# Chairy-neko/TinyRayTracing

Hardware: AMD Instinct MI355X
Metric: Mrays/s (higher is better)
Workload: dtype f32; 1 GPU; example-scenes-cg22 test/back Cornell-style box (26 triangles), 1920x1080, 256 spp; scene=back, width=1920, height=1080, spp=256, triangles=26, bvh_nodes=4, bvh_builder=auto, leaf_num=8, inner_node_bytes=64, overlap_passes=False, fixed_nee=False, tiling=single GPU

## Files before the change

tinyraytracing_amd/csrc/trt_api.hip:

```cpp
#include <hip/hip_runtime.h>

#include <dlfcn.h>

#include <algorithm>
#include <cstdio>
#include <cstdlib>
#include <atomic>
#include <limits>
#include <chrono>
#include <cstring>
#include <condition_variable>
#include <memory>
#include <mutex>
#include <string>
#include <thread>
#include <vector>

#include "trt.h"
#include "trt_kernels.h"
#include "trt_wide.h"
#include "trt_oct_build.h"
#include "trt_denoise_kernels.h"
#include "trt_reproject_kernels.h"
#include "trt_refit_kernels.h"
// ... 18 lines not shown
    } while (0)

constexpr uint32_t MAX_TRACE_BLOCKS = 8192;
constexpr uint32_t SPILL_STRIDE = MAX_TRACE_BLOCKS * TRT_TRACE_BLOCK;
constexpr uint32_t MAX_BOUNCES = TRT_MAX_PATH_DEPTH + 2;
constexpr uint32_t COUNT_STRIDE = (MAX_BOUNCES + 2 + 1023u) & ~1023u;
constexpr uint32_t COUNT_ROW_MIN = 16;
inline uint32_t countRows(uint32_t nl) { return std::max(COUNT_ROW_MIN, (nl + 3u + 15u) & ~15u); }
inline unsigned long long* pairCounter(uint32_t* d_counts, uint32_t rows, uint32_t b) { return reinterpret_cast<unsigned long long*>(d_counts + (size_t)(rows - 2u) * COUNT_STRIDE) + b; }
static_assert(TRT_MAX_SCENE_LIGHTS <= 65535u, "counter area");
constexpr uint32_t MAX_BVH_DEPTH = 256;
#ifndef TRT_DEFAULT_NODE_KIND
#define TRT_DEFAULT_NODE_KIND 1
#endif

struct DevBuf {
    void* p = nullptr;
    size_t bytes = 0;
    int ensure(size_t need)
    {
        if (need <= bytes) return TRT_OK;
        if (p) { (void)hipFree(p); p = nullptr; bytes = 0; }
        HIPC(hipMalloc(&p, need));
        bytes = need;
        return TRT_OK;
    }
    void release()
    {
        if (p) (void)hipFree(p);
        p = nullptr;
        bytes = 0;
    }
};

}

struct trt_handle {
    int device = 0;
    SceneDev sc{};
    std::vector<void*> scene_allocs;
    std::vector<uint32_t> light_mats;
    std::vector<LightBox> light_boxes;
    uint32_t depth = 0;
    uint32_t bvh2_depth = 0;
    uint32_t shade_tabs = 0;
    uint32_t shade_pad_lds = 0;
    const void* lds_image = nullptr;
    uint32_t lds_image_bytes = 0;
    uint32_t lds_tab[5] = {0, 0, 0, 0, 0};
    int trace_impl = 3;
    bool slim_walk = false;
    bool hit8 = false;
    bool bin_walk = false;
    int node_kind = 0;
    uint32_t oct_levels = 0;
    bool dbg = false;
    uint32_t rays_per_wave = 256, fill_blocks = 2048, max_blocks = 8192;
    uint32_t traceGrid(uint32_t n) const
    {
        uint32_t b = (n + TRT_TRACE_BLOCK - 1) / TRT_TRACE_BLOCK;
        if (rays_per_wave > 64) {
            const uint32_t want = (uint32_t)(((uint64_t)n + 4ull * rays_per_wave - 1) / (4ull * rays_per_wave));
            b = std::min(b, std::max(fill_blocks, want));
        }
        b = std::min(std::max(b, 8u), std::min(max_blocks, 8192u));
        return (b + 7u) & ~7u;
    }
    uint32_t tail_n = 131072;
    DevBuf arena, spill, small_buf, out_buf, io_buf;
    size_t spill_words_per_slot = 0;
    hipStream_t slot_streams[2] = {nullptr, nullptr};
    int n_slots = 2;
    uint32_t* pinned_counts = nullptr;
    uint32_t count_rows = COUNT_ROW_MIN;
    uint32_t slot_seq[2] = {0, 0};
    int fail_at_bounce = -1;
    std::vector<hipEvent_t> events;
    uint32_t n_materials = 0, n_light_tris = 0, n_tri_trav = 0;
    bool light_boxes_fixed = false;
    struct Refit {
        bool ready = false;
        DevBuf order2, order4, order8, exact8, small;
        std::vector<uint32_t> level2, level4, level8;
        DevBuf light_of_mat;
        hipEvent_t ev[4] = {};
    } refit;
    ~trt_handle()
    {
        refit.order2.release();
        refit.order4.release();
        refit.order8.release();
        refit.exact8.release();
        refit.small.release();
        refit.light_of_mat.release();
        for (hipEvent_t e : refit.ev)
            if (e) (void)hipEventDestroy(e);
        for (void* p : scene_allocs) (void)hipFree(p);
        arena.release();
        spill.release();
        small_buf.release();
        out_buf.release();
        io_buf.release();
        for (hipEvent_t e : events) (void)hipEventDestroy(e);
        for (hipStream_t st : slot_streams) if (st) (void)hipStreamDestroy(st);
        if (pinned_counts) (void)hipHostFree(pinned_counts);
    }
// ... 169 lines not shown
using ShadeKernel = void (*)(SceneDev, ShadeArgs);
using TailKernel = void (*)(SceneDev, TailArgs);

enum Walk { WALK_UNIFORM, WALK_UNIFORM_FLAGS, WALK_UNIFORM_HIT8, WALK_OCT, WALK_WIDE16, WALK_WIDE_SPILL, N_WALKS };
struct Traversal {
    Walk closest, occlusion;
    bool binned;
};
Traversal traversalOf(const trt_handle* h)
{
    if (h->trace_impl == 0) return {h->hit8 ? WALK_UNIFORM_HIT8 : WALK_UNIFORM, h->slim_walk ? WALK_UNIFORM_FLAGS : WALK_UNIFORM, h->bin_walk};
    const Walk w = h->node_kind == 1 ? WALK_OCT : (h->depth <= 16 ? WALK_WIDE16 : WALK_WIDE_SPILL);
    return {w, w, h->bin_walk};
}
struct ClosestRow { ClosestKernel k[2][3], query; bool redo; };
struct ShadowRow { ShadowKernel k[2]; ClosestKernel query; bool redo; };
template <class D>
ClosestRow closestRow()
{
    return {{{k_trace_closest<false, D, 0>, k_trace_closest<false, D, 1>, k_trace_closest<false, D, PRIMARY_LIST>},
             {k_trace_closest<true, D, 0>, k_trace_closest<true, D, 1>, k_trace_closest<true, D, PRIMARY_LIST>}},
            k_trace_query<D, QUERY_CLOSEST>, D::REDO};
}
template <class D>
ShadowRow shadowRow()
{
    return {{k_trace_shadow<false, D>, k_trace_shadow<true, D>}, k_trace_query<D, QUERY_OCCLUDED>, D::REDO};
}
const ClosestRow closest_rows[N_WALKS] = {closestRow<WalkUniform>(), {}, closestRow<WalkUniformHit8>(), closestRow<WalkOct>(), closestRow<WalkWide16>(), closestRow<WalkWideSpill>()};
const ShadowRow shadow_rows[N_WALKS] = {shadowRow<WalkUniform>(), shadowRow<WalkUniformFlags>(), {}, shadowRow<WalkOct>(), shadowRow<WalkWide16>(), shadowRow<WalkWideSpill>()};
ClosestKernel closestKernel(const trt_handle* h, bool count, int primary)
{
    const Traversal t = traversalOf(h);
    if (t.binned && primary == 0) return count ? k_trace_closest_binned<true> : k_trace_closest_binned<false>;
    return closest_rows[t.closest].k[count][primary];
}
ShadowKernel shadowKernel(const trt_handle* h, bool count) { return shadow_rows[traversalOf(h).occlusion].k[count]; }
FixKernel fixKernel(const trt_handle* h, bool shadow, int primary)
{
    const FixKernel k[4] = {k_trace_fix<false, 0>, k_trace_fix<false, 1>, k_trace_fix<false, PRIMARY_LIST>, k_trace_fix<true, 0>};
    const Traversal t = traversalOf(h);
    return (shadow ? shadow_rows[t.occlusion].redo : closest_rows[t.closest].redo) ? k[shadow ? 3 : primary] : nullptr;
}
ClosestKernel queryKernel(const trt_handle* h, int query)
{
    const Traversal t = traversalOf(h);
    return query == QUERY_OCCLUDED ? shadow_rows[t.occlusion].query : closest_rows[t.closest].query;
}
FixKernel queryFixKernel(const trt_handle* h, int query)
{
    if (!fixKernel(h, query == QUERY_OCCLUDED, 0)) return nullptr;
    return query == QUERY_OCCLUDED ? k_trace_fix<true, 0, QUERY_OCCLUDED> : k_trace_fix<false, 0, QUERY_CLOSEST>;
}
ShadeKernel shadeKernel(uint32_t tabs, int lights, bool list, bool hit8)
{
    if (hit8) {
        const ShadeKernel s[2][3] = {
            {k_shade<31u, SHADE_ONE, false, TRT_SHADE1_BLOCK, TRT_SHADE1_WAVES, true>, k_shade<31u, SHADE_FEW, false, TRT_SHADEN_BLOCK, TRT_SHADEN_WAVES, true>,
             k_shade<31u, SHADE_MANY, false, TRT_SHADEN_BLOCK, TRT_SHADEN_WAVES, true>},
            {k_shade<31u, SHADE_ONE, true, TRT_SHADE1_BLOCK, TRT_SHADE1_WAVES, true>, k_shade<31u, SHADE_FEW, true, TRT_SHADEN_BLOCK, TRT_SHADEN_WAVES, true>,
             k_shade<31u, SHADE_MANY, true, TRT_SHADEN_BLOCK, TRT_SHADEN_WAVES, true>}};
        return s[list][lights];
    }
    const ShadeKernel k[5][2][3] = {
        {{k_shade<31u, SHADE_ONE>, k_shade<31u, SHADE_FEW>, k_shade<31u, SHADE_MANY>}, {k_shade<31u, SHADE_ONE, true>, k_shade<31u, SHADE_FEW, true>, k_shade<31u, SHADE_MANY, true>}},
        {{k_shade<15u, SHADE_ONE>, k_shade<15u, SHADE_FEW>, k_shade<15u, SHADE_MANY>}, {k_shade<15u, SHADE_ONE, true>, k_shade<15u, SHADE_FEW, true>, k_shade<15u, SHADE_MANY, true>}},
        {{k_shade<7u, SHADE_ONE>, k_shade<7u, SHADE_FEW>, k_shade<7u, SHADE_MANY>}, {k_shade<7u, SHADE_ONE, true>, k_shade<7u, SHADE_FEW, true>, k_shade<7u, SHADE_MANY, true>}},
        {{k_shade<3u, SHADE_ONE>, k_shade<3u, SHADE_FEW>, k_shade<3u, SHADE_MANY>}, {k_shade<3u, SHADE_ONE, true>, k_shade<3u, SHADE_FEW, true>, k_shade<3u, SHADE_MANY, true>}},
        {{k_shade<0u, SHADE_ONE>, k_shade<0u, SHADE_FEW>, k_shade<0u, SHADE_MANY>}, {k_shade<0u, SHADE_ONE, true>, k_shade<0u, SHADE_FEW, true>, k_shade<0u, SHADE_MANY, true>}}};
    return k[tabs == 31u ? 0 : (tabs == 15u ? 1 : (tabs == 7u ? 2 : (tabs == 3u ? 3 : 4)))][list][lights];
}
TailKernel tailKernel(bool count, bool list)
{
    if (list) return count ? k_tail<true, true> : k_tail<false, true>;
    return count ? k_tail<true> : k_tail<false>;
}

void launchTraceClosest(const trt_handle* h, ClosestKernel k, FixKernel fix, hipStream_t stream, uint32_t* spill, const RaySource& src, f4* hit, uint32_t n,
                        DeviceStats* d_stats, RedoList redo)
{
    const dim3 b(TRT_TRACE_BLOCK);
    hipLaunchKernelGGL(k, dim3(h->traceGrid(n)), b, 0, stream, h->sc, src, hit, n, spill, SPILL_STRIDE, d_stats, redo);
    if (fix) hipLaunchKernelGGL(fix, dim3(TRT_FIX_BLOCKS), b, 0, stream, h->sc, src, hit, (const f4*)nullptr, 0u, (f4*)nullptr, spill, SPILL_STRIDE, redo, 0u, d_stats);
}

void launchTraceShadow(const trt_handle* h, ShadowKernel k, FixKernel fix, hipStream_t stream, uint32_t* spill, const ShadowQueue& sq, uint32_t n, uint32_t light_mat,
                       f4* Lacc, DeviceStats* d_stats, uint32_t any, RedoList redo, const LightBox& lbox)
{
    const dim3 b(TRT_TRACE_BLOCK);
    hipLaunchKernelGGL(k, dim3(h->traceGrid(n)), b, 0, stream, h->sc, sq, n, light_mat, Lacc, spill, SPILL_STRIDE, d_stats, any, redo, lbox);
    if (!fix) return;
    const RaySource src{sq.sa, sq.sb, TileDesc{}, 0u};
    hipLaunchKernelGGL(fix, dim3(TRT_FIX_BLOCKS), b, 0, stream, h->sc, src, (f4*)nullptr, (const f4*)sq.sw, light_mat, Lacc, spill, SPILL_STRIDE, redo, any, d_stats);
}

}

namespace {
struct SceneImage {
    const trt_scene* s = nullptr;
    unsigned threads = 1;
    bool dbg = false;
    uint32_t bvh2_depth = 0;
    int trace_impl = 3;
    int node_kind = 0;
    std::vector<TriIsect> isect;
// ... 206 lines not shown
    if (im.cum_monotone)
        if (int e = upload(h.get(), im.cum.data(), im.cum.size(), &h->sc.light_cum)) return e;
    if (int e = upload(h.get(), im.tex.data(), im.tex.size(), &h->sc.textures)) return e;
    if (int e = upload(h.get(), im.tex_bytes.data(), im.tex_bytes.size(), &h->sc.tex_bytes)) return e;
    lap("uploads");
    h->sc.n_tris = s->n_tris;
    h->sc.n_nodes = s->n_nodes;
    h->sc.n_lights = s->n_lights;
    h->n_materials = s->n_materials;
    h->n_light_tris = s->n_light_tris;
    if (const char* e = std::getenv("TRT_SHADOW_STOP")) h->light_boxes_fixed = std::atoi(e) == 0;
    h->sc.light0_area = s->n_lights ? s->lights[0].area : 0.0f;
    h->sc.leaf_alpha = im.leaf_alpha;
    h->sc.cull_alpha = im.cull_alpha;
    h->sc.cam = s->camera;
    for (uint32_t i = 0; i < s->n_lights; ++i) h->light_mats.push_back((uint32_t)s->lights[i].mat);
    {
        const uint32_t want[5] = {(uint32_t)(s->n_materials * sizeof(MaterialDev)), (uint32_t)(s->n_lights * sizeof(LightDev)),
                                  h->sc.light_cum ? (uint32_t)(s->n_light_tris * sizeof(float)) : 0u, (uint32_t)(s->n_light_tris * sizeof(LightTriDev)),
                                  s->n_tris <= 64 ? (uint32_t)(s->n_tris * sizeof(TriShade)) : 0u};
        uint32_t used = 0;
        for (int k = 0; k < 5; ++k) {
            const uint32_t padded = (want[k] + 15u) & ~15u;
            if (want[k] && used + padded <= TRT_SHADE_LDS_TABLE_BYTES) { h->lds_tab[k] = want[k]; used += padded; }
        }
        if (std::getenv("TRT_SHADE_NO_LDS")) h->lds_tab[0] = h->lds_tab[1] = h->lds_tab[2] = h->lds_tab[3] = h->lds_tab[4] = 0;
        if (std::getenv("TRT_SHADE_NO_LDS_TRIS")) h->lds_tab[4] = 0;
        uint32_t have = 0;
        for (int k = 0; k < 5; ++k) have |= h->lds_tab[k] ? (1u << k) : 0u;
        h->shade_tabs = 0;
        for (uint32_t m : {31u, 15u, 7u, 3u})
            if ((have & m) == m) { h->shade_tabs = m; break; }
        if (im.dbg)
            std::fprintf(stderr, "trt_create: k_shade tables %u (lds bytes: materials %u, lights %u, cdf %u, light tris %u, shading tris %u)\n", h->shade_tabs,
                         h->lds_tab[0], h->lds_tab[1], h->lds_tab[2], h->lds_tab[3], h->lds_tab[4]);
        size_t total = 0;
        for (int k = 0; k < 5; ++k)
            if (h->shade_tabs >> k & 1u) total += (h->lds_tab[k] + 15u) & ~15u;
        if (total) {
            void* img = nullptr;
            HIPC(hipMalloc(&img, total));
            h->scene_allocs.push_back(img);
            h->lds_image = img;
            h->lds_image_bytes = (uint32_t)total;
            if (int e = packLdsImage(h.get(), nullptr)) return e;
        }
    }
    h->slim_walk = h->trace_impl == 0 && s->n_tris <= 64;
    if (const char* e = std::getenv("TRT_SLIM_WALK")) h->slim_walk = h->slim_walk && std::atoi(e) != 0;
    h->hit8 = h->slim_walk && h->shade_tabs == 31u;
    h->bin_walk = h->hit8;
    if (const char* e = std::getenv("TRT_BIN_WALK")) h->bin_walk = h->bin_walk && std::atoi(e) != 0;
    if (im.dbg) std::fprintf(stderr, "trt_create: slim walk %d, 8-byte hit records %d, binned walk %d\n", (int)h->slim_walk, (int)h->hit8, (int)h->bin_walk);

    const uint32_t stack_levels = std::max(h->depth, h->bvh2_depth + 2u);
    uint32_t spill_levels = stack_levels > (uint32_t)TRT_LDS_STACK_MAX ? stack_levels - TRT_LDS_STACK_MAX + 1 : 1;
    if (h->node_kind == 1 && h->oct_levels > OCT_LDS_LEVELS) spill_levels = std::max(spill_levels, 2u * (h->oct_levels - OCT_LDS_LEVELS + 1));
    h->spill_words_per_slot = (size_t)spill_levels * SPILL_STRIDE;
    if (int e = h->spill.ensure(h->spill_words_per_slot * 2 * sizeof(uint32_t))) return e;
    for (hipStream_t& st : h->slot_streams) HIPC(hipStreamCreateWithFlags(&st, hipStreamNonBlocking));
    h->count_rows = countRows(h->sc.n_lights);
    const size_t pinned_words = 2 * (2 * (size_t)h->count_rows + 16);
    HIPC(hipHostMalloc((void**)&h->pinned_counts, pinned_words * sizeof(uint32_t), hipHostMallocDefault));
    std::memset(h->pinned_counts, 0, pinned_words * sizeof(uint32_t));
    if (const char* e = std::getenv("TRT_SLOTS")) h->n_slots = std::atoi(e) >= 2 ? 2 : 1;
    if (const char* e = std::getenv("TRT_TEST_FAIL_AT_BOUNCE")) h->fail_at_bounce = std::atoi(e);
    if (const char* e = std::getenv("TRT_SHADE_PAD_LDS")) {
        h->shade_pad_lds = std::min(100000u, (uint32_t)std::strtoul(e, nullptr, 10));
        for (uint32_t tabs : {31u, 15u, 7u, 3u, 0u})
            for (bool list : {false, true})
                for (int lights : {SHADE_ONE, SHADE_FEW, SHADE_MANY})
                    for (bool hit8 : {false, true})
                        if (!hit8 || tabs == 31u)
                            (void)hipFuncSetAttribute(reinterpret_cast<const void*>(shadeKernel(tabs, lights, list, hit8)), hipFuncAttributeMaxDynamicSharedMemorySize, (int)h->shade_pad_lds);
    }

    *out = h.release();
    return TRT_OK;
}
}

extern "C" {

const char* trt_last_error(void) { return g_err.c_str(); }
int trt_abi_version(void) { return TRT_ABI_VERSION; }

int trt_rows_selected(const trt_params* p)
{
    if (!p) return -1;
    int n = 0;
    for (int y = p->y0; y < p->y1; ++y) n += rowSelected(p, y) ? 1 : 0;
    return n;
}

int trt_create(const trt_scene* s, int device, trt_handle** out)
{
    if (!s || !out) return fail(TRT_EINVAL, "trt_create: null argument");
    *out = nullptr;
    SceneImage im;
    if (int e = buildSceneImage(s, im)) return e;
    return createOnDevice(im, device, out);
}

void trt_destroy(trt_handle* h)
{
    if (!h) return;
    (void)hipSetDevice(h->device);
    delete h;
}

namespace {
constexpr int N_SLOTS = 2;
struct PassSlot {
    hipStream_t stream = nullptr;
    RayQueue Q[2];
    f4* hit = nullptr;
    f4* Lacc = nullptr;
    ShadowArena shadow{nullptr, 0};
    uint32_t* d_counts = nullptr;
    uint32_t* host_counts = nullptr;
    uint32_t seq = 0;
    uint32_t* spill = nullptr;
    RedoList redo{nullptr, nullptr};
    enum State { IDLE, PACK, PACKWAIT, ISSUE, WAIT, RESOLVE } state = IDLE;
    uint32_t chunk = 0, s0 = 0, sc_count = 0, n_active = 0, b = 0;
    int cur = 0;
};
// ... 203 lines not shown
        if (d_sq) HIPC(hipMemcpyAsync(d_sq, in.sumsq, acc_bytes, hipMemcpyHostToDevice, stream));
    }
    if (!in.list || in.rays) return TRT_OK;
    uint32_t list_max = 0;
    hipLaunchKernelGGL(k_list_max, dim3(std::min<uint32_t>((in.npix + 255) / 256, 1024u)), dim3(256), 0, stream, in.host ? (const uint32_t*)d_table : in.pixels, in.npix, d_list_max);
    HIPC(hipMemcpyAsync(&list_max, d_list_max, sizeof(list_max), hipMemcpyDeviceToHost, stream));
    HIPC(hipStreamSynchronize(stream));
    if ((uint64_t)list_max >= (uint64_t)p->width * (uint64_t)p->height) return fail(TRT_EINVAL, "pixel list holds an entry >= width * height");
    return TRT_OK;
}

int renderCore(trt_handle* h, const trt_params* p, uint32_t s_begin, uint32_t s_end, const RenderInput& in, hipStream_t stream, trt_stats* stats_out)
{
    const uint32_t n_samples = s_end - s_begin, npix = in.npix, nl = h->sc.n_lights, count_rows = h->count_rows;
    PassPlan plan;
    if (int e = planArena(h, p, npix, n_samples, in.list, renderFootprint(nl), plan)) return e;
    const size_t counts_bytes = (size_t)COUNT_STRIDE * count_rows * sizeof(uint32_t), acc_bytes = (size_t)npix * 3 * sizeof(double);
    const bool own_table = in.host || (in.rays && !in.pixels);
    const size_t table_bytes = !own_table ? 0 : (in.list ? (size_t)npix * sizeof(uint32_t) : in.rows.size() * sizeof(int32_t));
    Layout L;
    const size_t o_table = L.add(table_bytes, 256), o_counts = L.add(counts_bytes * N_SLOTS, 256);
    const size_t o_stats = L.add(sizeof(DeviceStats), 256), o_redo = L.add(2 * N_SLOTS * sizeof(uint32_t), 64), o_list_max = L.add(sizeof(uint32_t), 64);
    const size_t o_pack = L.add(N_SLOTS * sizeof(unsigned long long), 64);
    const size_t o_sum = L.add(in.host ? acc_bytes : 0, 256), o_sumsq = L.add(in.host && in.sumsq ? acc_bytes : 0, sizeof(double));
    if (int e = h->small_buf.ensure(L.bytes)) return e;
    char* sb = (char*)h->small_buf.p;
    DeviceStats* d_stats = (DeviceStats*)(sb + o_stats);
    const void* d_table = own_table ? (const void*)(sb + o_table) : (const void*)in.pixels;
    double* d_sum = in.host ? (double*)(sb + o_sum) : in.sum;
    double* d_sq = !in.sumsq ? nullptr : (in.host ? (double*)(sb + o_sumsq) : in.sumsq);
    HIPC(hipMemsetAsync(d_stats, 0, o_sum - o_stats, stream));
    if (int e = stageInput(in, p, sb + o_table, table_bytes, d_sum, d_sq, (uint32_t*)(sb + o_list_max), stream)) return e;
    PassSlot slots[N_SLOTS];
    for (int k = 0; k < plan.slots; ++k) {
        PassSlot& S = slots[k];
        S.stream = h->slot_streams[k];
        SlotLayout::carve(S, (f4*)((char*)h->arena.p + plan.slot_bytes * (size_t)k), plan.N, nl);
        S.redo.count = (uint32_t*)(sb + o_redo) + 2 * k;
        S.d_counts = (uint32_t*)(sb + o_counts + counts_bytes * (size_t)k);
        S.host_counts = h->pinned_counts + (size_t)k * (2 * count_rows + 16);
        S.seq = h->slot_seq[k];
        S.spill = (uint32_t*)h->spill.p + (size_t)k * h->spill_words_per_slot;
    }
    const int lights = nl == 1u ? SHADE_ONE : (nl <= (uint32_t)TRT_MAX_LIGHTS ? SHADE_FEW : SHADE_MANY);
    const uint32_t shade_block = lights == SHADE_ONE ? (uint32_t)TRT_SHADE1_BLOCK : (uint32_t)TRT_SHADEN_BLOCK;
    const uint32_t rows_lds = (in.rows.size() <= shadeRowsLds((int)shade_block) && p->height <= 65536) ? (uint32_t)in.rows.size() : 0u;
    const bool count = (p->flags & TRT_FLAG_COUNT) != 0;
    const int camera = in.list ? PRIMARY_LIST : 1;
    const ClosestKernel camera_k = closestKernel(h, count, camera), queue_k = closestKernel(h, count, 0);
    const FixKernel camera_fix = fixKernel(h, false, camera), queue_fix = fixKernel(h, false, 0), shadow_fix = fixKernel(h, true, 0);
    const ShadowKernel shadow_k = shadowKernel(h, count);
    const ShadeKernel shade_k = shadeKernel(h->shade_tabs, lights, in.list, h->hit8);
    const TailKernel tail_k = tailKernel(count, in.list);
    const ShadeArgs shade_args = shadeArgsOf(h, p, in, d_table, rows_lds, d_stats);
    const TileDesc& td = shade_args.td;
    if (h->dbg)
        std::fprintf(stderr, "%s: k_shade %s, rows in lds %u, grid_ok %u\n", in.rays ? "trt_render_rays" : (in.list ? "trt_render_pixels" : "trt_render"),
                     lights == SHADE_ONE ? "one" : (lights == SHADE_FEW ? "few" : "many"), rows_lds, td.grid_ok);

    Timer tm{h, (p->flags & TRT_FLAG_TIMING) != 0};
    trt_stats st;
    std::memset(&st, 0, sizeof(st));
    hipEvent_t ev_begin = tm.get(0), ev_end = tm.get(1), ev_resolved = tm.get(2);
    if (!ev_begin || !ev_end || !ev_resolved) return fail(TRT_EHIP, "hipEventCreate failed");
    HIPC(hipEventRecord(ev_begin, stream));
    Drain drain{h, slots, plan.slots, stream};
    for (int k = 0; k < plan.slots; ++k) HIPC(hipStreamWaitEvent(slots[k].stream, ev_begin, 0));

    uint32_t next_chunk = 0, resolved_upto = 0;
    auto startPass = [&](PassSlot& S) -> int {
        if (next_chunk >= plan.n_chunks) { S.state = PassSlot::IDLE; return TRT_OK; }
        S.chunk = next_chunk++;
        S.s0 = s_begin + S.chunk * plan.chunk;
        S.sc_count = std::min(plan.chunk, s_end - S.s0);
        S.n_active = npix * S.sc_count;
        S.b = 0;
        S.cur = 0;
        HIPC(hipMemsetAsync(S.d_counts, 0, counts_bytes, S.stream));
        if (!in.rays) st.rays_camera += S.n_active;
        S.state = in.rays ? PassSlot::PACK : PassSlot::ISSUE;
        return TRT_OK;
    };
    auto issuePack = [&](PassSlot& S) -> int {
        const size_t at = (size_t)(S.s0 - s_begin) * npix * 3, comps = (size_t)S.n_active * 3;
        const float* org = in.org + at;
        const float* dir = in.dir + at;
        if (in.host) {
            float* stage = (float*)S.Q[1].ra;
            HIPC(hipMemcpyAsync(stage, org, comps * sizeof(float), hipMemcpyHostToDevice, S.stream));
            HIPC(hipMemcpyAsync(stage + comps, dir, comps * sizeof(float), hipMemcpyHostToDevice, S.stream));
            org = stage;
            dir = stage + comps;
        }
        unsigned long long* packed = (unsigned long long*)(sb + o_pack) + (&S - slots);
        HIPC(hipMemsetAsync(packed, 0, sizeof(*packed), S.stream));
        tm.launch(TRT_K_GEN_PRIMARY, S.stream, st, [&] {
            hipLaunchKernelGGL(k_rays_pack, dim3(std::min<uint32_t>((S.n_active + 255) / 256, 65536u)), dim3(256), 0, S.stream, org, dir, S.n_active, S.Q[0], S.Lacc,
                               (uint32_t*)packed);
        });
        S.seq++;
        hipLaunchKernelGGL(k_publish_counts, dim3(1), dim3(64), 0, S.stream, S.d_counts, COUNT_STRIDE, 0u, 1u, packed, (volatile uint32_t*)S.host_counts, 2u * count_rows, S.seq);
        S.state = PassSlot::PACKWAIT;
        return TRT_OK;
    };
    auto completePack = [&](PassSlot& S) -> int {
        if (int e = awaitCounts(S, count_rows)) return e;
        const uint32_t n_valid = S.host_counts[1];
        if (n_valid > S.n_active) return fail(TRT_EHIP, "internal error: more rays queued than given");
        st.rays_camera += n_valid;
        S.n_active = n_valid;
        S.state = n_valid ? PassSlot::ISSUE : PassSlot::RESOLVE;
        return TRT_OK;
    };
    auto issueFront = [&](PassSlot& S) -> int {
        const RaySource src{S.Q[S.cur].ra, S.Q[S.cur].rb, td, S.s0};
        tm.launch(TRT_K_TRACE_CLOSEST, S.stream, st, [&] {
            const bool generated = S.b == 0 && !in.rays;
            launchTraceClosest(h, generated ? camera_k : queue_k, generated ? camera_fix : queue_fix, S.stream, S.spill, src, S.hit, S.n_active, d_stats, S.redo);
        });
        ShadeArgs A = shade_args;
        A.qin = S.Q[S.cur];
        A.hit = S.hit;
        A.n = S.n_active;
        A.qout = S.Q[S.cur ^ 1];
        if (lights == SHADE_MANY) A.sq_arena = S.shadow;
        else
            for (uint32_t l = 0; l < (uint32_t)TRT_MAX_LIGHTS; ++l) A.sq[l] = l < nl ? S.shadow.queue(l) : ShadowQueue{nullptr, nullptr, nullptr};
        A.pair_count = pairCounter(S.d_counts, count_rows, S.b);
        A.shadow_counts = S.d_counts + (size_t)COUNT_STRIDE + S.b;
        A.Lacc = S.Lacc;
        A.s0 = S.s0;
        A.primary = (S.b == 0 && !in.rays) ? 1u : 0u;
        tm.launch(TRT_K_SHADE, S.stream, st, [&] {
            hipLaunchKernelGGL(shade_k, dim3(std::min<uint32_t>((S.n_active + shade_block - 1) / shade_block, 65536u)), dim3(shade_block), h->shade_pad_lds, S.stream, h->sc, A);
        });
        S.seq++;
        const uint32_t publish_block = std::min(1024u, (2u * (1u + nl) + 63u) & ~63u);
        hipLaunchKernelGGL(k_publish_counts, dim3(1), dim3(publish_block), 0, S.stream, S.d_counts, COUNT_STRIDE, S.b, 1u + nl,
                           pairCounter(S.d_counts, count_rows, S.b), (volatile uint32_t*)S.host_counts, 2u * count_rows, S.seq);
        S.state = PassSlot::WAIT;
        if (h->fail_at_bounce >= 0 && (int)S.b == h->fail_at_bounce) {
            h->fail_at_bounce = -1;
            return fail(TRT_EHIP, "injected failure (TRT_TEST_FAIL_AT_BOUNCE)");
        }
        return TRT_OK;
    };
    auto completeBounce = [&](PassSlot& S) -> int {
        if (int e = awaitCounts(S, count_rows)) return e;
        for (uint32_t l = 0; l < nl; ++l) {
            const uint32_t ns = S.host_counts[2 * (1 + l)];
            if (ns > S.n_active) return fail(TRT_EHIP, "internal error: shadow queue longer than its input");
            if (!ns) continue;
            tm.launch(TRT_K_TRACE_SHADOW, S.stream, st, [&] {
                launchTraceShadow(h, shadow_k, shadow_fix, S.stream, S.spill, S.shadow.queue(l), ns, h->light_mats[l], S.Lacc, d_stats, td.fixed_nee, S.redo, h->light_boxes[l]);
            });
            st.rays_shadow += ns;
        }
        const uint32_t n_next = S.host_counts[1];
        if (n_next > S.n_active) return fail(TRT_EHIP, "internal error: queue grew");
        st.rays_indirect += n_next;
        S.n_active = n_next;
        S.cur ^= 1;
        S.b++;
        if (S.n_active > 0 && (S.n_active <= h->tail_n || S.b >= MAX_BOUNCES)) {
            const TailArgs TA{S.Q[S.cur], S.n_active, S.Lacc, td, S.s0, p->max_depth, S.spill, SPILL_STRIDE, h->trace_impl == 0 ? 1u : 0u, d_stats};
            tm.launch(TRT_K_TAIL, S.stream, st, [&] { hipLaunchKernelGGL(tail_k, dim3(tailGrid(S.n_active)), dim3(TRT_TRACE_BLOCK), 0, S.stream, h->sc, TA); });
            S.n_active = 0;
        }
        S.state = S.n_active ? PassSlot::ISSUE : PassSlot::RESOLVE;
        return TRT_OK;
    };
    auto tryResolve = [&](PassSlot& S) -> int {
        if (S.chunk != resolved_upto) return TRT_OK;
        if (resolved_upto > 0) HIPC(hipStreamWaitEvent(S.stream, ev_resolved, 0));
        tm.launch(TRT_K_RESOLVE, S.stream, st, [&] {
            const dim3 rg(std::min<uint32_t>((npix + 255) / 256, 65536u)), rb(256);
            if (d_sq) hipLaunchKernelGGL(k_resolve_moments, rg, rb, 0, S.stream, S.Lacc, d_sum, d_sq, npix, S.sc_count, (float)p->spp);
            else hipLaunchKernelGGL(k_resolve, rg, rb, 0, S.stream, S.Lacc, d_sum, npix, S.sc_count, (float)p->spp);
        });
        HIPC(hipEventRecord(ev_resolved, S.stream));
        resolved_upto++;
        return startPass(S);
    };

    for (int k = 0; k < plan.slots; ++k)
        if (int e = startPass(slots[k])) return e;
    for (;;) {
// ... 1432 lines not shown
```

tinyraytracing_amd/csrc/trt_kernels.h:

```cpp
#pragma once
#include <hip/hip_runtime.h>
#include <type_traits>

#include "trt_path.h"
#include "trt_oct.h"

namespace trtd {

#ifndef TRT_TRACE_MINWAVES
#define TRT_TRACE_MINWAVES 0
#endif
#if TRT_TRACE_MINWAVES > 0
#define TRT_TRACE_BOUNDS __launch_bounds__(256, TRT_TRACE_MINWAVES)
#else
#define TRT_TRACE_BOUNDS __launch_bounds__(256)
#endif
constexpr int TRT_TRACE_BLOCK = 256;
#ifndef TRT_LDS_STACK_MAX_LEVELS
#define TRT_LDS_STACK_MAX_LEVELS 16
#endif
constexpr int TRT_LDS_STACK_MAX = TRT_LDS_STACK_MAX_LEVELS;
#ifndef TRT_SHADE1_BLOCK
#define TRT_SHADE1_BLOCK 512
#endif
// ... 1028 lines not shown
    uint32_t n;
    RayQueue qout;
    union {
        ShadowQueue sq[TRT_MAX_LIGHTS];
        ShadowArena sq_arena;
    };
    unsigned long long* pair_count;
    uint32_t* shadow_counts;
    uint32_t shadow_count_stride;
    f4* Lacc;
    TileDesc td;
    uint32_t s0;
    int32_t max_depth;
    uint32_t primary;
    uint32_t lds_mat_bytes, lds_light_bytes, lds_cum_bytes, lds_ltri_bytes, lds_tshade_bytes;
    const f4* lds_image;
    uint32_t lds_image_words;
    uint32_t rows_lds;
    DeviceStats* stats;
};

constexpr uint32_t TRT_SHADE_LDS_TABLE_BYTES = 24 * 1024;
constexpr uint32_t shadeRowsLds(int block) { return block >= 512 ? 8192u : 2304u; }

struct RowsShade {
    const uint16_t* lds;
    bool in_lds;
    __device__ int operator()(const TileDesc& td, uint32_t r) const
    {
        int y = 0;
        if (in_lds) {
            y = lds[r];
#if defined(__HIP_DEVICE_COMPILE__)
            asm volatile("" : "+v"(y));
#endif
        } else {
            y = td.rows[r];
        }
        return y;
    }
};

__device__ __forceinline__ void hitBarycentrics(const TriIsect* isect, const f4& ra, const f4& rb, f4& hit4)
{
    const int32_t tri = (int32_t)f2u(hit4.y);
    float u = 0.f, v = 0.f;
    if (tri >= 0) {
        float t, un, vn, det;
        if (triTest(isect[tri], mk3(ra.x, ra.y, ra.z), mk3(ra.w, rb.x, rb.y), t, un, vn, det)) { u = un / det; v = vn / det; }
    }
    hit4.z = u;
    hit4.w = v;
}
template <int LIGHTS>
__device__ inline ShadowQueue shadeQueue(const ShadeArgs& A, uint32_t li)
{
    if (LIGHTS == SHADE_MANY) return A.sq_arena.queue(li);
    return A.sq[li];
}
template <uint32_t TABS, int LIGHTS, bool LIST = false, int BLOCK = (LIGHTS == SHADE_ONE ? TRT_SHADE1_BLOCK : TRT_SHADEN_BLOCK),
          int WAVES = (LIGHTS == SHADE_ONE ? TRT_SHADE1_WAVES : TRT_SHADEN_WAVES), bool HIT8 = false>
__global__ __launch_bounds__(BLOCK, WAVES) void k_shade(SceneDev sc, ShadeArgs A)
{
    constexpr int TRT_SHADE_BLOCK = BLOCK;
    constexpr uint32_t TRT_SHADE_ROWS_LDS = shadeRowsLds(BLOCK);
    __shared__ uint32_t s_cnt[3 * (TRT_SHADE_BLOCK / 64 + 1)];
    __shared__ uint32_t s_cnt2[2 * (2 * (TRT_SHADE_BLOCK / 64) + 2)];
    __shared__ uint32_t s_shaded, s_depth;
    __shared__ __attribute__((aligned(16))) uint32_t s_tab[TABS ? TRT_SHADE_LDS_TABLE_BYTES / 4 : 4];
    __shared__ uint16_t s_rows[LIST ? 1 : TRT_SHADE_ROWS_LDS];
    __shared__ __attribute__((aligned(16))) uint32_t s_isect[HIT8 ? 64 * 12 : 4];
    const TriIsect* isect = reinterpret_cast<const TriIsect*>(s_isect);
    if (threadIdx.x == 0) { s_shaded = 0; s_depth = 0; }
    if (!LIST)
        for (uint32_t r = threadIdx.x; r < A.rows_lds; r += TRT_SHADE_BLOCK) s_rows[r] = (uint16_t)A.td.rows[r];
    std::conditional_t<LIST, PixelList, RowsShade> rows;
    if constexpr (!LIST) {
        rows.lds = s_rows;
        rows.in_lds = A.rows_lds != 0u;
    }
    bool rows_visible = A.rows_lds == 0u;
    {
        uint32_t off = 0;
        auto at = [&](uint32_t bytes) -> const void* { const void* q = s_tab + off / 4; off += (bytes + 15u) & ~15u; return q; };
        if (TABS & 1u) sc.materials = static_cast<const MaterialDev*>(at(A.lds_mat_bytes));
        if (TABS & 2u) sc.lights = static_cast<const LightDev*>(at(A.lds_light_bytes));
        if (TABS & 4u) sc.light_cum = static_cast<const float*>(at(A.lds_cum_bytes));
        if (TABS & 8u) sc.light_tris = static_cast<const LightTriDev*>(at(A.lds_ltri_bytes));
        if (TABS & 16u) sc.tri_shade = static_cast<const TriShade*>(at(A.lds_tshade_bytes));
    }
    bool staged = TABS == 0u && !HIT8;
    int parity = 0, parity2 = 0;
    uint32_t bounce_depth = 0;
    const uint32_t per_grid = gridDim.x * TRT_SHADE_BLOCK;
    auto loadTile = [&](uint32_t i, f4& hit4, f4& ra, f4& rb, f4& bt) {
        hit4 = mk4(TRT_INF, u2f(0xFFFFFFFFu), 0.0f, 0.0f); ra = mk4(0, 0, 0, 0); rb = ra; bt = mk4(1.0f, 1.0f, 1.0f, 0.0f);
        if (i < A.n) {
            if (HIT8) {
                const trt_v2f h = TRT_LDQ2(1, reinterpret_cast<const trt_v2f*>(A.hit) + i);
                hit4.x = h.x; hit4.y = h.y;
            } else {
                hit4 = TRT_LDQ(1, A.hit + i);
            }
            if (!A.primary) { ra = TRT_LDQ(1, A.qin.ra + i); rb = TRT_LDQ(1, A.qin.rb + i); bt = TRT_LDQ(1, A.qin.bt + i); }
        }
    };
#if TRT_SHADE_PIPE
    f4 n_hit, n_ra, n_rb, n_bt;
    loadTile(blockIdx.x * TRT_SHADE_BLOCK + threadIdx.x, n_hit, n_ra, n_rb, n_bt);
#endif
    for (uint32_t base = blockIdx.x * TRT_SHADE_BLOCK; base < A.n; base += per_grid) {
        const uint32_t i = base + threadIdx.x;
        f4 hit4, ra, rb, bt;
#if TRT_SHADE_PIPE
        hit4 = n_hit; ra = n_ra; rb = n_rb; bt = n_bt;
#else
        loadTile(i, hit4, ra, rb, bt);
#endif
        if (!staged || !rows_visible) {
            if (!staged) {
                f4* l = reinterpret_cast<f4*>(s_tab);
                if (TABS)
                    for (uint32_t w = threadIdx.x; w < A.lds_image_words; w += TRT_SHADE_BLOCK) l[w] = A.lds_image[w];
                if (HIT8) {
                    f4* li = reinterpret_cast<f4*>(s_isect);
                    const uint32_t words = 3u * (sc.n_tris < 64u ? sc.n_tris : 64u);
                    for (uint32_t w = threadIdx.x; w < words; w += TRT_SHADE_BLOCK) li[w] = reinterpret_cast<const f4*>(sc.tri_isect)[w];
                }
            }
            __syncthreads();
            staged = true;
            rows_visible = true;
        }
#if defined(__HIP_DEVICE_COMPILE__)
        asm volatile("" : "+v"(hit4.x), "+v"(ra.x), "+v"(rb.x), "+v"(bt.x));
#endif
#if TRT_SHADE_PIPE
        loadTile(i + per_grid, n_hit, n_ra, n_rb, n_bt);
#endif
        ShadeCtx c;
        c.had_hit = c.shade_ok = c.add_L = false;
        if (i < A.n) {
            if (A.primary) {
                primaryRay(sc, A.td, A.s0, i, ra, rb, rows);
                if (HIT8) hitBarycentrics(isect, ra, rb, hit4);
                shadeBegin(sc, A.td, A.s0, ra, rb, bt, hit4, c, rows);
                A.Lacc[i] = c.add_L ? mk4(0.0f + c.addL.x, 0.0f + c.addL.y, 0.0f + c.addL.z, 0.0f) : mk4(0.0f, 0.0f, 0.0f, 0.0f);
            } else {
                if (HIT8) hitBarycentrics(isect, ra, rb, hit4);
                shadeBegin(sc, A.td, A.s0, ra, rb, bt, hit4, c, rows);
                if (c.add_L) {
                    f4 L = A.Lacc[c.pid];
                    L.x = L.x + c.addL.x; L.y = L.y + c.addL.y; L.z = L.z + c.addL.z;
                    A.Lacc[c.pid] = L;
                }
            }
            if (c.had_hit) bounce_depth = c.depth + 1u > bounce_depth ? c.depth + 1u : bounce_depth;
        }
        const unsigned long long ok_ballot = ballotb(c.shade_ok);
        if ((threadIdx.x & 63u) == 0 && ok_ballot) atomicAdd(&s_shaded, (uint32_t)__popcll(ok_ballot));

        uint32_t pend_base = 0;
        const uint32_t* pend_s = nullptr;
        bool pend_emit = false;
        uint32_t pend_rank = 0, pend_li = 0;
        f3 pend_wo = mk3(0, 0, 0), pend_w = mk3(0, 0, 0);
        float pend_tmax = TRT_INF;
        const uint32_t nl = LIGHTS == SHADE_ONE ? 1u : sc.n_lights;
        for (uint32_t li = 0; li + 1 < nl; ++li) {
            bool emit = false;
            f3 wo = mk3(0, 0, 0), contrib = mk3(0, 0, 0);
            float t_max = TRT_INF;
            if (c.shade_ok) emit = lightSample(sc, c.vx, *c.m, li, c.rng, wo, contrib, A.td.fixed_nee != 0u, t_max);
            uint32_t rank;
            uint32_t* s = blockStage<TRT_SHADE_BLOCK>(emit, A.shadow_counts + (size_t)li * A.shadow_count_stride, s_cnt, parity, rank, pend_s, pend_base);
            parity = parity == 2 ? 0 : parity + 1;
            if (pend_emit) {
                const uint32_t slot = pend_s[TRT_SHADE_BLOCK / 64] + pend_s[threadIdx.x >> 6] + pend_rank;
                const f3 so = rayOrigin(c, pend_wo);
                TRT_STQ(2, shadeQueue<LIGHTS>(A, pend_li).sa + slot, mk4(so.x, so.y, so.z, pend_wo.x));
                TRT_STQ(2, shadeQueue<LIGHTS>(A, pend_li).sb + slot, mk4(pend_wo.y, pend_wo.z, u2f(c.pid), pend_tmax));
                TRT_STQ(2, shadeQueue<LIGHTS>(A, pend_li).sw + slot, mk4(pend_w.x, pend_w.y, pend_w.z, 0.0f));
            }
            pend_s = s; pend_emit = emit; pend_rank = rank; pend_li = li; pend_wo = wo; pend_w = c.beta * contrib; pend_tmax = t_max;
        }
        bool emit_s = false;
        f3 wo_s = mk3(0, 0, 0), w_s = mk3(0, 0, 0);
        float tmax_s = TRT_INF;
        if (nl && c.shade_ok) {
            f3 contrib = mk3(0, 0, 0);
            emit_s = lightSample(sc, c.vx, *c.m, nl - 1u, c.rng, wo_s, contrib, A.td.fixed_nee != 0u, tmax_s);
            w_s = c.beta * contrib;
        }
        NextPlan plan;
        const bool emit_next = shadeNextDecide(c, A.max_depth, plan);
        uint32_t rank_next, rank_s;
// ... 454 lines not shown
```

Measured before the change: 23940 Mrays/s.

## Fuse primary-ray closest-hit traversal into the bounce-0 shade kernel

For single-light scenes on the slim 8-byte-hit path, bounce 0 no longer launches a separate closest-hit trace kernel. The shade kernel regenerates the camera ray, walks the small BVH itself with a wave-uniform reachability mask, and shades the hit directly. This removes one kernel launch per pass along with the hit-buffer write and read round trip. In exchange it adds traversal register pressure to the shade kernel, and it reads triangles from global memory instead of the LDS copy.

```diff
diff --git a/tinyraytracing_amd/csrc/trt_api.hip b/tinyraytracing_amd/csrc/trt_api.hip
--- a/tinyraytracing_amd/csrc/trt_api.hip
+++ b/tinyraytracing_amd/csrc/trt_api.hip
@@ -94,6 +94,7 @@
     bool slim_walk = false;
     bool hit8 = false;
     bool bin_walk = false;
+    bool fuse_primary = false;
     int node_kind = 0;
     uint32_t oct_levels = 0;
     bool dbg = false;
@@ -369,6 +370,7 @@
     if (!fixKernel(h, query == QUERY_OCCLUDED, 0)) return nullptr;
     return query == QUERY_OCCLUDED ? k_trace_fix<true, 0, QUERY_OCCLUDED> : k_trace_fix<false, 0, QUERY_CLOSEST>;
 }
+ShadeKernel fusedShadeKernel() { return k_shade<31u, SHADE_ONE, false, TRT_SHADE1_BLOCK, TRT_SHADE1_WAVES, true, true>; }
 ShadeKernel shadeKernel(uint32_t tabs, int lights, bool list, bool hit8)
 {
     if (hit8) {
@@ -681,6 +683,9 @@
     h->bin_walk = h->hit8;
     if (const char* e = std::getenv("TRT_BIN_WALK")) h->bin_walk = h->bin_walk && std::atoi(e) != 0;
     if (im.dbg) std::fprintf(stderr, "trt_create: slim walk %d, 8-byte hit records %d, binned walk %d\n", (int)h->slim_walk, (int)h->hit8, (int)h->bin_walk);
+    h->fuse_primary = h->hit8 && s->n_lights == 1;
+    if (const char* e = std::getenv("TRT_FUSE_PRIMARY")) h->fuse_primary = h->fuse_primary && std::atoi(e) != 0;
+    if (im.dbg) std::fprintf(stderr, "trt_create: fused primary %d\n", (int)h->fuse_primary);
 
     const uint32_t stack_levels = std::max(h->depth, h->bvh2_depth + 2u);
     uint32_t spill_levels = stack_levels > (uint32_t)TRT_LDS_STACK_MAX ? stack_levels - TRT_LDS_STACK_MAX + 1 : 1;
@@ -702,6 +707,7 @@
                     for (bool hit8 : {false, true})
                         if (!hit8 || tabs == 31u)
                             (void)hipFuncSetAttribute(reinterpret_cast<const void*>(shadeKernel(tabs, lights, list, hit8)), hipFuncAttributeMaxDynamicSharedMemorySize, (int)h->shade_pad_lds);
+        (void)hipFuncSetAttribute(reinterpret_cast<const void*>(fusedShadeKernel()), hipFuncAttributeMaxDynamicSharedMemorySize, (int)h->shade_pad_lds);
     }
 
     *out = h.release();
@@ -1011,11 +1017,13 @@
     const ShadowKernel shadow_k = shadowKernel(h, count);
     const ShadeKernel shade_k = shadeKernel(h->shade_tabs, lights, in.list, h->hit8);
     const TailKernel tail_k = tailKernel(count, in.list);
+    const bool fuse = h->fuse_primary && lights == SHADE_ONE && !in.list && !in.rays && !count;
     const ShadeArgs shade_args = shadeArgsOf(h, p, in, d_table, rows_lds, d_stats);
     const TileDesc& td = shade_args.td;
     if (h->dbg)
         std::fprintf(stderr, "%s: k_shade %s, rows in lds %u, grid_ok %u\n", in.rays ? "trt_render_rays" : (in.list ? "trt_render_pixels" : "trt_render"),
                      lights == SHADE_ONE ? "one" : (lights == SHADE_FEW ? "few" : "many"), rows_lds, td.grid_ok);
+    if (h->dbg) std::fprintf(stderr, "%s: fused primary %d\n", in.rays ? "trt_render_rays" : (in.list ? "trt_render_pixels" : "trt_render"), (int)fuse);
 
     Timer tm{h, (p->flags & TRT_FLAG_TIMING) != 0};
     trt_stats st;
@@ -1073,10 +1081,12 @@
     };
     auto issueFront = [&](PassSlot& S) -> int {
         const RaySource src{S.Q[S.cur].ra, S.Q[S.cur].rb, td, S.s0};
-        tm.launch(TRT_K_TRACE_CLOSEST, S.stream, st, [&] {
-            const bool generated = S.b == 0 && !in.rays;
-            launchTraceClosest(h, generated ? camera_k : queue_k, generated ? camera_fix : queue_fix, S.stream, S.spill, src, S.hit, S.n_active, d_stats, S.redo);
-        });
+        const bool generated = S.b == 0 && !in.rays;
+        const bool fused = fuse && generated;
+        if (!fused)
+            tm.launch(TRT_K_TRACE_CLOSEST, S.stream, st, [&] {
+                launchTraceClosest(h, generated ? camera_k : queue_k, generated ? camera_fix : queue_fix, S.stream, S.spill, src, S.hit, S.n_active, d_stats, S.redo);
+            });
         ShadeArgs A = shade_args;
         A.qin = S.Q[S.cur];
         A.hit = S.hit;
@@ -1091,7 +1101,8 @@
         A.s0 = S.s0;
         A.primary = (S.b == 0 && !in.rays) ? 1u : 0u;
         tm.launch(TRT_K_SHADE, S.stream, st, [&] {
-            hipLaunchKernelGGL(shade_k, dim3(std::min<uint32_t>((S.n_active + shade_block - 1) / shade_block, 65536u)), dim3(shade_block), h->shade_pad_lds, S.stream, h->sc, A);
+            hipLaunchKernelGGL(fused ? fusedShadeKernel() : shade_k, dim3(std::min<uint32_t>((S.n_active + shade_block - 1) / shade_block, 65536u)), dim3(shade_block),
+                               h->shade_pad_lds, S.stream, h->sc, A);
         });
         S.seq++;
         const uint32_t publish_block = std::min(1024u, (2u * (1u + nl) + 63u) & ~63u);
diff --git a/tinyraytracing_amd/csrc/trt_kernels.h b/tinyraytracing_amd/csrc/trt_kernels.h
--- a/tinyraytracing_amd/csrc/trt_kernels.h
+++ b/tinyraytracing_amd/csrc/trt_kernels.h
@@ -1104,6 +1104,79 @@
     hit4.z = u;
     hit4.w = v;
 }
+template <bool GLM>
+__device__ __forceinline__ void fusedWalk(const SceneDev& sc, f3 o, f3 d, f3 inv, bool special, float& best_t, int32_t& best_tri, float& best_un,
+                                          float& best_vn, float& best_det)
+{
+    const uint32_t n_nodes = sc.n_nodes;
+    uint32_t reach = 1u;
+    uint32_t best_flags = 0u;
+    for (uint32_t ni = 0; ni < n_nodes; ++ni) {
+        const bool at = (reach >> ni) & 1u;
+        if (ballotb(at) == 0ull) continue;
+        const f4* np4 = reinterpret_cast<const f4*>(sc.nodes + ni);
+        const f4 q0 = np4[0], q1 = np4[1], q2 = np4[2], q3 = np4[3];
+        float e0 = 0.0f, e1 = 0.0f;
+        bool h0 = at && boxTest(q0.x, q0.y, q0.z, q0.w, q1.x, q1.y, o, inv, e0);
+        bool h1 = at && boxTest(q1.z, q1.w, q2.x, q2.y, q2.z, q2.w, o, inv, e1);
+        if (GLM) {
+            float g0, g1;
+            const bool s0 = boxTestGlm(q0.x, q0.y, q0.z, q0.w, q1.x, q1.y, o, inv, g0), s1 = boxTestGlm(q1.z, q1.w, q2.x, q2.y, q2.z, q2.w, o, inv, g1);
+            if (special) { h0 = at && s0; h1 = at && s1; e0 = g0; e1 = g1; }
+        }
+        const float f0 = trt_leaf_floor(e0, sc.leaf_alpha), f1 = trt_leaf_floor(e1, sc.leaf_alpha);
+        const uint32_t child[2] = {f2u(q3.x), f2u(q3.y)};
+        const bool hc[2] = {h0, h1};
+#pragma unroll
+        for (int c = 0; c < 2; ++c) {
+            const uint32_t ref = child[c];
+            if (!(ref & TRT_LEAF_BIT)) {
+                reach |= hc[c] ? (1u << ref) : 0u;
+                continue;
+            }
+            if (ballotb(hc[c]) == 0ull) continue;
+            const uint32_t first = TRT_LEAF_FIRST(ref), count = TRT_LEAF_COUNT(ref);
+            for (uint32_t k = 0; k < count; ++k) {
+                const TriIsect T = sc.tri_isect[first + k];
+                float tn, un, vn, det;
+                bool ok_det, ok_in;
+                triCandidateParts(T, o, d, tn, un, vn, det, ok_det, ok_in);
+                if (ok_det && ok_in && hc[c]) {
+                    const float t = tn / det;
+                    if (!(t < TRT_T_MIN) && !(t < (c == 0 ? f0 : f1))) {
+                        const int32_t j = (int32_t)(first + k);
+                        const uint32_t fl = f2u(T.c.z);
+                        bool take = t < best_t;
+                        if (t == best_t && best_tri >= 0) {
+                            const bool em = (fl & 1u) != 0, bem = (best_flags & 1u) != 0;
+                            const bool same_leaf = (uint32_t)best_tri >= first && (uint32_t)best_tri < first + count;
+                            take = same_leaf ? em : (em ? (!bem || j < best_tri) : (!bem && j > best_tri));
+                        }
+                        if (take) { best_t = t; best_tri = j; best_flags = fl; best_un = un; best_vn = vn; best_det = det; }
+                    }
+                }
+            }
+        }
+    }
+}
+__device__ __forceinline__ f4 fusedPrimaryHit(const SceneDev& sc, const f4& ra, const f4& rb, DeviceStats* stats)
+{
+    const f3 o = mk3(ra.x, ra.y, ra.z), d = mk3(ra.w, rb.x, rb.y);
+    const f3 inv = mk3(1.0f / d.x, 1.0f / d.y, 1.0f / d.z);
+    const bool special = raySpecial(inv);
+    float best_t = TRT_INF, un = 0.0f, vn = 0.0f, det = 1.0f;
+    int32_t best_tri = -1;
+    const unsigned long long m_sp = ballotb(special);
+    if (m_sp != 0ull) {
+        fusedWalk<true>(sc, o, d, inv, special, best_t, best_tri, un, vn, det);
+        if ((threadIdx.x & 63u) == 0) atomicAdd(&stats->redo_rays, (uint32_t)__popcll(m_sp));
+    } else {
+        fusedWalk<false>(sc, o, d, inv, false, best_t, best_tri, un, vn, det);
+    }
+    float u = 0.0f, v = 0.0f;
+    if (best_tri >= 0) { u = un / det; v = vn / det; }
+    return mk4(best_t, u2f((uint32_t)best_tri), u, v);
+}
 template <int LIGHTS>
 __device__ inline ShadowQueue shadeQueue(const ShadeArgs& A, uint32_t li)
 {
@@ -1111,9 +1184,10 @@
     return A.sq[li];
 }
 template <uint32_t TABS, int LIGHTS, bool LIST = false, int BLOCK = (LIGHTS == SHADE_ONE ? TRT_SHADE1_BLOCK : TRT_SHADEN_BLOCK),
-          int WAVES = (LIGHTS == SHADE_ONE ? TRT_SHADE1_WAVES : TRT_SHADEN_WAVES), bool HIT8 = false>
+          int WAVES = (LIGHTS == SHADE_ONE ? TRT_SHADE1_WAVES : TRT_SHADEN_WAVES), bool HIT8 = false, bool FUSE = false>
 __global__ __launch_bounds__(BLOCK, WAVES) void k_shade(SceneDev sc, ShadeArgs A)
 {
+    static_assert(!FUSE || (HIT8 && !LIST && LIGHTS == SHADE_ONE), "the fused bounce 0 is built for tile renders of one-light scenes of the wave-uniform walk");
     constexpr int TRT_SHADE_BLOCK = BLOCK;
     constexpr uint32_t TRT_SHADE_ROWS_LDS = shadeRowsLds(BLOCK);
     __shared__ uint32_t s_cnt[3 * (TRT_SHADE_BLOCK / 64 + 1)];
@@ -1121,7 +1195,7 @@
     __shared__ uint32_t s_shaded, s_depth;
     __shared__ __attribute__((aligned(16))) uint32_t s_tab[TABS ? TRT_SHADE_LDS_TABLE_BYTES / 4 : 4];
     __shared__ uint16_t s_rows[LIST ? 1 : TRT_SHADE_ROWS_LDS];
-    __shared__ __attribute__((aligned(16))) uint32_t s_isect[HIT8 ? 64 * 12 : 4];
+    __shared__ __attribute__((aligned(16))) uint32_t s_isect[HIT8 && !FUSE ? 64 * 12 : 4];
     const TriIsect* isect = reinterpret_cast<const TriIsect*>(s_isect);
     if (threadIdx.x == 0) { s_shaded = 0; s_depth = 0; }
     if (!LIST)
@@ -1147,6 +1221,7 @@
     const uint32_t per_grid = gridDim.x * TRT_SHADE_BLOCK;
     auto loadTile = [&](uint32_t i, f4& hit4, f4& ra, f4& rb, f4& bt) {
         hit4 = mk4(TRT_INF, u2f(0xFFFFFFFFu), 0.0f, 0.0f); ra = mk4(0, 0, 0, 0); rb = ra; bt = mk4(1.0f, 1.0f, 1.0f, 0.0f);
+        if (FUSE) return;
         if (i < A.n) {
             if (HIT8) {
                 const trt_v2f h = TRT_LDQ2(1, reinterpret_cast<const trt_v2f*>(A.hit) + i);
@@ -1174,7 +1249,7 @@
                 f4* l = reinterpret_cast<f4*>(s_tab);
                 if (TABS)
                     for (uint32_t w = threadIdx.x; w < A.lds_image_words; w += TRT_SHADE_BLOCK) l[w] = A.lds_image[w];
-                if (HIT8) {
+                if (HIT8 && !FUSE) {
                     f4* li = reinterpret_cast<f4*>(s_isect);
                     const uint32_t words = 3u * (sc.n_tris < 64u ? sc.n_tris : 64u);
                     for (uint32_t w = threadIdx.x; w < words; w += TRT_SHADE_BLOCK) li[w] = reinterpret_cast<const f4*>(sc.tri_isect)[w];
@@ -1185,7 +1260,7 @@
             rows_visible = true;
         }
 #if defined(__HIP_DEVICE_COMPILE__)
-        asm volatile("" : "+v"(hit4.x), "+v"(ra.x), "+v"(rb.x), "+v"(bt.x));
+        if (!FUSE) asm volatile("" : "+v"(hit4.x), "+v"(ra.x), "+v"(rb.x), "+v"(bt.x));
 #endif
 #if TRT_SHADE_PIPE
         loadTile(i + per_grid, n_hit, n_ra, n_rb, n_bt);
@@ -1193,7 +1268,12 @@
         ShadeCtx c;
         c.had_hit = c.shade_ok = c.add_L = false;
         if (i < A.n) {
-            if (A.primary) {
+            if (FUSE) {
+                primaryRay(sc, A.td, A.s0, i, ra, rb, rows);
+                hit4 = fusedPrimaryHit(sc, ra, rb, A.stats);
+                shadeBegin(sc, A.td, A.s0, ra, rb, bt, hit4, c, rows);
+                A.Lacc[i] = c.add_L ? mk4(0.0f + c.addL.x, 0.0f + c.addL.y, 0.0f + c.addL.z, 0.0f) : mk4(0.0f, 0.0f, 0.0f, 0.0f);
+            } else if (A.primary) {
                 primaryRay(sc, A.td, A.s0, i, ra, rb, rows);
                 if (HIT8) hitBarycentrics(isect, ra, rb, hit4);
                 shadeBegin(sc, A.td, A.s0, ra, rb, bt, hit4, c, rows);
```

Result: faster. 24790 Mrays/s (median of 6 runs) (+3.6%).
